# shamspias/fennec

Hardware: AMD Instinct MI355X
Metric: megapixels/sec: 4K SSIMFast+GaussianBlur (higher is better)
Workload: dtype u8 (blur: exact int32 sums of 24-bit fixed-point weights on the i8 matrix pipe; fp64 SSIM)

## Files before the change

fennec_amd/csrc/blur.hip:

```cpp
#include <hip/hip_ext.h>

#include "common.hpp"
#include "devutil.hpp"

#include <algorithm>
#include <cmath>

namespace fnx {

template <typename T>
struct PassArgs {
    const uint8_t *src;
    const uint8_t *const *srcs;
    const uint8_t *alpha;
    const uint8_t *const *alphas;
    uint8_t *dst;
    uint8_t *const *dsts;
    int sstride, astride, dstride, w, h, radius;
    const T *kern;
};

template <typename T> __device__ __forceinline__ T acc_tap(T acc, uint32_t v, T wt);
template <> __device__ __forceinline__ double acc_tap<double>(double acc, uint32_t v, double wt)
{
// ... 638 lines not shown

static bool guard_kernel_ok(const double *kernel, int radius)
{
    double sum = 0;
    for (int i = 0; i < 2 * radius + 1; i++) {
        if (!(kernel[i] >= 0)) return false;
        sum += kernel[i];
    }
    return sum <= 1.0 + 1e-9;
}

template <int R, bool SCORE, bool GUARD = false>
static int launch_direct(fnx_ctx *ctx, int n, FusedArgs &fa, bool tall)
{
    if constexpr (R > SCORE_RMAX) {
        static_assert(!SCORE, "one-pass form: R <= 8");
        return launch_direct_cfg<R, 256, WIDE_IH, false, GUARD>(ctx, n, fa);
    } else {
        constexpr int TH0 = ((64 - 2 * R) / 4) * 4;
        if (tall) return launch_direct_cfg<R, 256, 2 * TH0 + 2 * R, SCORE, GUARD>(ctx, n, fa);
        return launch_direct_cfg<R, 128, 64, SCORE, GUARD>(ctx, n, fa);
    }
}

template <bool SCORE, bool GUARD = false>
static int launch_direct_radius(fnx_ctx *ctx, int radius, int n, FusedArgs &fa, bool tall)
{
    switch (radius) {
    case 1: return launch_direct<1, SCORE, GUARD>(ctx, n, fa, tall);
    case 2: return launch_direct<2, SCORE, GUARD>(ctx, n, fa, tall);
    case 3: return launch_direct<3, SCORE, GUARD>(ctx, n, fa, tall);
    case 4: return launch_direct<4, SCORE, GUARD>(ctx, n, fa, tall);
    case 5: return launch_direct<5, SCORE, GUARD>(ctx, n, fa, tall);
    case 6: return launch_direct<6, SCORE, GUARD>(ctx, n, fa, tall);
    case 7: return launch_direct<7, SCORE, GUARD>(ctx, n, fa, tall);
    case 8: return launch_direct<8, SCORE, GUARD>(ctx, n, fa, tall);
    }
    if constexpr (!SCORE) {
        switch (radius) {
        case 9: return launch_direct<9, false, GUARD>(ctx, n, fa, tall);
        case 10: return launch_direct<10, false, GUARD>(ctx, n, fa, tall);
        case 11: return launch_direct<11, false, GUARD>(ctx, n, fa, tall);
        case 12: return launch_direct<12, false, GUARD>(ctx, n, fa, tall);
        case 13: return launch_direct<13, false, GUARD>(ctx, n, fa, tall);
        case 14: return launch_direct<14, false, GUARD>(ctx, n, fa, tall);
        case 15: return launch_direct<15, false, GUARD>(ctx, n, fa, tall);
        case 16: return launch_direct<16, false, GUARD>(ctx, n, fa, tall);
        }
    }
    return FNX_ERR_INVALID;
}

constexpr int NHEAD = 260 + 257 * 8;
static bool build_score_geom(fnx::ScoreGeom &g, int w, int h, int radius, int dstW, int dstH, int th_fixed = 0)
{
    if (radius < 1 || radius > (th_fixed ? 24 : SCORE_RMAX) || w < dstW || h < dstH || dstW <= 0 || dstH <= 0 || w >= (1 << 24) ||
        h >= (1 << 24))
        return false;
    const double xr = static_cast<double>(w) / static_cast<double>(dstW);
    const double yr = static_cast<double>(h) / static_cast<double>(dstH);
    if (std::fmin(xr, yr) < 3.6) return false;
    const size_t ref_words = 4 * (static_cast<size_t>(dstW) + dstH);
    std::vector<int32_t> &map = g.map;
    map.assign(NHEAD + ref_words + static_cast<size_t>(w) + h, -1);
    {
        uint32_t *magic = reinterpret_cast<uint32_t *>(map.data()), *tiedown = magic + 260;
        std::fill(magic, magic + NHEAD, 0u);
        for (uint32_t c = 1; c <= 256; c++) {
            magic[c] = static_cast<uint32_t>((1ull << 32) / (2ull * c)) + 1u;
            if (c & 1u) continue;
            const double inv = 1.0 / static_cast<double>(c);
            for (uint32_t k = 0; k < 256; k++) {
                const double n = static_cast<double>(c / 2) * static_cast<double>(2 * k + 1);
                if (n > 255.0 * c) break;
                if (n * inv < static_cast<double>(k) + 0.5) tiedown[8 * c + (k >> 5)] |= 1u << (k & 31);
            }
        }
    }
    BoxRef *xref = reinterpret_cast<BoxRef *>(map.data() + NHEAD), *yref = xref + dstW;
    int32_t *bx = map.data() + NHEAD + ref_words, *by = bx + w;
    int maxbw = 0, maxbh = 0;
    for (int d = 0; d < dstW; d++) {
        int s0, s1;
        box_edge(d, xr, w, s0, s1);
        if (d + 1 < dstW) { int n0, n1; box_edge(d + 1, xr, w, n0, n1); if (n0 < s1) return false; }
        for (int x = s0; x < s1; x++) bx[x] = d;
        if (s1 - s0 > maxbw) maxbw = s1 - s0;
    }
    for (int d = 0; d < dstH; d++) {
        int s0, s1;
        box_edge(d, yr, h, s0, s1);
        if (d + 1 < dstH) { int n0, n1; box_edge(d + 1, yr, h, n0, n1); if (n0 < s1) return false; }
        for (int y = s0; y < s1; y++) by[y] = d;
        if (s1 - s0 > maxbh) maxbh = s1 - s0;
    }
    if (static_cast<long>(maxbw) * maxbh > 256) return false;
    bool tall = g.tall_pref;
    int th = 0, nbx = 0, nby = 0;
    for (int attempt = 0; attempt < (th_fixed ? 1 : 2); attempt++, tall = !tall) {
        th = th_fixed ? th_fixed : direct_tile_rows(radius, tall);
        nbx = nby = 1;
        auto span = [](const int32_t *m, int lo, int hi) {
            int first = -1, last = -1;
            for (int i = lo; i < hi; i++)
                if (m[i] >= 0) { if (first < 0) first = m[i]; last = m[i]; }
            return first < 0 ? 0 : last - first + 1;
        };
        for (int x0 = 0; x0 < w; x0 += 64) nbx = std::max(nbx, span(bx, x0, std::min(w, x0 + 64)));
        for (int y0 = 0; y0 < h; y0 += th) nby = std::max(nby, span(by, y0, std::min(h, y0 + th)));
        if ((nbx + 1) * (nby + 1) <= (th_fixed > 272 ? 2 * SCORE_NBOX : SCORE_NBOX)) break;
        th = 0;
    }
    if (!th) return false;
    tall = th == direct_tile_rows(radius, true);
    if (th_fixed) {
        for (int x0 = 0; x0 < w; x0 += 16) {
            int first = -1, last = -1;
            for (int x = x0; x < std::min(w, x0 + 16); x++)
                if (bx[x] >= 0) { if (first < 0) first = bx[x]; last = bx[x]; }
            if (first >= 0 && last - first > 4) return false;
        }
    }
    for (int x0 = 0; x0 < w; x0 += 64)
        if (bx[x0] < 0) for (int x = x0; x < std::min(w, x0 + 64); x++) if (bx[x] >= 0) return false;
    for (int y0 = 0; y0 < h; y0 += th)
        if (by[y0] < 0) for (int y = y0; y < std::min(h, y0 + th); y++) if (by[y] >= 0) return false;

    const int slabn = (nbx + 1) * (nby + 1);
    const int tiles_x = (w + 63) / 64, tiles = tiles_x * ((h + th - 1) / th);
    if (static_cast<size_t>(tiles) * 2 * slabn >= (1u << 30)) return false;
    for (int d = 0; d < dstW; d++) {
        int s0, s1;
        box_edge(d, xr, w, s0, s1);
        const int t0 = s0 >> 6, t1 = (s1 - 1) >> 6;
        if (t1 > t0 + 1) return false;
        xref[d].part0 = t0 * 2 * slabn + (d - bx[t0 << 6]);
        xref[d].part1 = t1 > t0 ? t1 * 2 * slabn + (d - bx[t1 << 6]) : -1;
        xref[d].len = s1 - s0; xref[d].pad = 0;
    }
    for (int d = 0; d < dstH; d++) {
        int s0, s1;
        box_edge(d, yr, h, s0, s1);
        const int t0 = s0 / th, t1 = (s1 - 1) / th;
        if (t1 > t0 + 1) return false;
        yref[d].part0 = t0 * tiles_x * 2 * slabn + (d - by[t0 * th]) * (nbx + 1);
        yref[d].part1 = t1 > t0 ? t1 * tiles_x * 2 * slabn + (d - by[t1 * th]) * (nbx + 1) : -1;
        yref[d].len = s1 - s0; yref[d].pad = 0;
    }

    g.th = th; g.nbx = nbx; g.nby = nby; g.tall = tall;
    return true;
}

int launch_blur_scored(fnx_ctx *ctx, int n, const uint8_t *const *srcs, int sstride, int w, int h,
                       const double *kernel, int radius, int flags, uint8_t *const *dsts, int dstride,
                       uint8_t *planes, size_t plane, int dstW, int dstH)
{
    if (n > 65535) return FNX_NOOP;
    const bool exact = flags & FNX_BLUR_EXACT;
    const bool wide = radius > 6 && blur_mfma_wide_scored_covers(kernel, radius, w, h, exact);
    if (!wide) {
        if (radius < 1 || radius > SCORE_RMAX) return FNX_NOOP;
        if (exact && !guard_kernel_ok(kernel, radius)) return FNX_NOOP;
        if (radius > 6 && blur_mfma_takes(kernel, radius, w, h, exact)) return FNX_NOOP;
    }
    const bool tall_pref = wide ? false : direct_tall(ctx, radius, n, w, h);
    static const int wide_cap = [] { const char *e = dev_env("FNX_MFMA_WIDE_SEG"); return e ? atoi(e) : 544; }();
    const int seg = wide ? blur_mfma_segment(ctx, n, w, h, wide_cap, 2)
                         : (blur_mfma_covers(kernel, radius, w, h) && (!exact || blur_mfma_exact_enabled()) ? blur_mfma_segment(ctx, n, w, h, 272, 3) : 0);
    ScoreGeom &g = ctx->score_geom;
    if (!(g.w == w && g.h == h && g.dstW == dstW && g.dstH == dstH && g.radius == radius && g.tall_pref == tall_pref && g.seg == seg)) {
        g.w = w; g.h = h; g.dstW = dstW; g.dstH = dstH; g.radius = radius; g.tall_pref = tall_pref; g.seg = seg;
        g.mfma = seg > 0 && build_score_geom(g, w, h, radius, dstW, dstH, seg);
        g.ok = g.mfma || (!wide && seg == 0 && build_score_geom(g, w, h, radius, dstW, dstH));
    }
    if (!g.ok) return FNX_NOOP;
    const std::vector<int32_t> &map = g.map;
    const int th = g.th, nbx = g.nbx, nby = g.nby;
    const bool tall = g.tall;
    const size_t ref_words = 4 * (static_cast<size_t>(dstW) + dstH);
    const int slabn = (nbx + 1) * (nby + 1);
    const int tiles_x = (w + 63) / 64, tiles = tiles_x * ((h + th - 1) / th);

    void *dmap = nullptr;
    FNX_TRY(upload_table(ctx, SLOT_BOXMAP, map.data(), sizeof(int32_t) * map.size(), &dmap));
    FusedArgs fa{};
    fa.srcs = srcs; fa.dsts = dsts;
    fa.sstride = sstride; fa.dstride = dstride; fa.w = w; fa.h = h;
    for (int i = 0; i < 2 * radius + 1 && !wide; i++) {
        fa.wt[i] = static_cast<float>(kernel[i]);
        fa.wd[i] = kernel[i];
    }
    fa.bx = static_cast<const int32_t *>(dmap) + NHEAD + ref_words; fa.by = fa.bx + w;
    fa.nbx = nbx; fa.nby = nby;
    void *slabs = nullptr;
    FNX_TRY(scratch(ctx, ctx->parity ? SLOT_SLABS1 : SLOT_SLABS, sizeof(unsigned long long) * 2 * slabn * static_cast<size_t>(tiles) * n, &slabs));
    fa.slabs = static_cast<unsigned long long *>(slabs);
    int st;
    if (g.mfma) {
        st = wide ? launch_blur_mfma_wide_scored(ctx, n, srcs, sstride, w, h, kernel, radius, flags, dsts, dstride, fa.bx, fa.by, fa.slabs, nbx, nby, th)
                  : launch_blur_mfma_scored(ctx, n, srcs, sstride, w, h, kernel, radius, flags, dsts, dstride, fa.bx, fa.by, fa.slabs, nbx, nby, th);
        if (st == FNX_NOOP) return FNX_NOOP;
    } else {
        st = exact ? launch_direct_radius<true, true>(ctx, radius, n, fa, tall)
                   : launch_direct_radius<true, false>(ctx, radius, n, fa, tall);
    }
    if (st < 0) return st;
    hipStream_t box_stream = ctx->stream2;
    if (ctx->boxes_on_main) box_stream = ctx->stream;
    else {
        FNX_HIP(hipStreamWaitEvent(ctx->stream2, ctx->blur_done, 0));
        ctx->stream2_used = true;
    }

    SlabArgs sa{};
    sa.slabs = fa.slabs; sa.dst = planes; sa.plane = plane;
    sa.magic = static_cast<const uint32_t *>(dmap);
    sa.tiedown = sa.magic + 260;
    sa.xref = reinterpret_cast<const BoxRef *>(static_cast<const int32_t *>(dmap) + NHEAD);
    sa.yref = sa.xref + dstW;
    sa.image_slabs = static_cast<size_t>(tiles) * 2 * slabn;
    sa.n = n; sa.dstW = dstW; sa.dstH = dstH; sa.slabn = slabn;
    hipLaunchKernelGGL(box_from_slabs_kernel, dim3((dstW + 64 * BFS_BOXES - 1) / (64 * BFS_BOXES), (dstH + 3) / 4, n), dim3(256), 0,
                       box_stream, sa);
    FNX_HIP(hipGetLastError());
    return FNX_OK;
// ... 236 lines not shown
```

fennec_amd/csrc/blur_mfma.hip:

```cpp
#include <hip/hip_ext.h>

#include "common.hpp"
#include "devutil.hpp"

#include <algorithm>
#include <cmath>
#include <type_traits>
#include <vector>

namespace fnx {

typedef int v4i __attribute__((ext_vector_type(4)));

constexpr int MF_RMAX = 6;
constexpr int MF_P = 48;
constexpr int MF_WT = 64 * MF_P + 256;
constexpr int MF_SP = 352;
constexpr int MF_OP = 272;
constexpr int MF_SEG_SCORE = 272;
constexpr int MF_SEG_SCORE_WIDE = 544;

struct MfmaArgs {
    const uint8_t *src;
    const uint8_t *const *srcs;
    uint8_t *dst;
    uint8_t *const *dsts;
    int sstride, dstride, w, h;
    int tiles_x, tiles, seg;
    int radius;
    const uint32_t *tab;
    int seed_h, seed_v, thr;
    const int32_t *bx, *by;
    unsigned long long *slabs;
    int nbx, nby;
    int dbg;
};

__device__ __forceinline__ int mf_comb3(int hi, int mid, int lo)
{
    int t = hi * 256 + mid;
    asm volatile("" : "+v"(t));
    return t * 256 + lo;
}

__device__ __forceinline__ const double *mf_scalar_ptr(const double *p)
{
    const unsigned long long v = reinterpret_cast<unsigned long long>(p);
    const unsigned lo = __builtin_amdgcn_readfirstlane(static_cast<unsigned>(v)), hi = __builtin_amdgcn_readfirstlane(static_cast<unsigned>(v >> 32));
    return reinterpret_cast<const double *>((static_cast<unsigned long long>(hi) << 32) | lo);
}
typedef int mf_s16i __attribute__((ext_vector_type(16)));
__device__ __forceinline__ uint32_t mf_exact_u(const double *wd, const uint8_t *base, int step, int ring0, int mask)
{
    mf_s16i w0, w1;
    asm volatile("s_load_dwordx16 %0, %2, 0x0\n\ts_load_dwordx16 %1, %2, 0x40\n\ts_waitcnt lgkmcnt(0)" : "=&s"(w0), "=&s"(w1) : "s"(mf_scalar_ptr(wd)) : "memory");
    uint32_t v[13];
#pragma unroll
    for (int t = 0; t < 13; t++) v[t] = base[((ring0 + t) & mask) * step];
    double acc = 0;
#pragma unroll
    for (int t = 0; t < 13; t++) {
        const int lo = t < 8 ? w0[2 * (t & 7)] : w1[2 * (t & 7)], hi = t < 8 ? w0[2 * (t & 7) + 1] : w1[2 * (t & 7) + 1];
        acc = acc + u8_to_f64(v[t] ^ 0x80u) * __hiloint2double(hi, lo);
    }
    return clampF_dev(acc);
}

__device__ __forceinline__ void mf_box_add4(uint32_t *tbl, const u32x4 ro, uint32_t coln, const v4i cb)
{
#pragma unroll
    for (int k = 0; k < 4; k++)
        __hip_atomic_fetch_add(reinterpret_cast<uint32_t *>(reinterpret_cast<char *>(tbl) + ro[k] + coln), static_cast<uint32_t>(cb[k]),
                               __ATOMIC_RELAXED, __HIP_MEMORY_SCOPE_WORKGROUP);
}

template <bool SCORE, bool GUARD>
__global__ __launch_bounds__(256, GUARD ? 3 : 1) void blur_mfma_kernel(MfmaArgs a)
{
    constexpr int P = MF_P, WT = MF_WT, SP = MF_SP, OP = MF_OP;
    __shared__ __attribute__((aligned(16))) uint8_t s_t[4 * WT];
    __shared__ __attribute__((aligned(16))) uint8_t s_stage[2 * 16 * SP];
    __shared__ __attribute__((aligned(16))) uint8_t s_out[2 * 16 * OP];
    __shared__ __attribute__((aligned(16))) uint32_t s_rowh[SCORE ? MF_SEG_SCORE + 32 : 4];
    __shared__ __attribute__((aligned(16))) uint32_t s_rowv[SCORE ? MF_SEG_SCORE + 16 : 4];
    __shared__ uint32_t s_colbox[SCORE ? 64 : 1];
    extern __shared__ __attribute__((aligned(16))) uint32_t s_box[];

    const int tile = xcd_tile(blockIdx.x, a.tiles);
    if (tile < 0) return;
    const int z = blockIdx.y;
    const uint8_t *src = a.srcs ? a.srcs[z] : a.src;
    uint8_t *dst = a.dsts ? a.dsts[z] : a.dst;
    const int ty = tile / a.tiles_x, tx = tile - ty * a.tiles_x;
    const int x0 = tx * 64, y0 = ty * a.seg;
    const int tid = threadIdx.x, wave = tid >> 6, lane = tid & 63;
    const int r = lane & 15, g = lane >> 4;
    const int NJ = min(a.seg, ((a.h - y0 + 15) >> 4) << 4) >> 4;
    const int NI = NJ + 1;
    const bool xedge = x0 - 6 < 0 || x0 + 70 > a.w;

    const v4i *tbh = reinterpret_cast<const v4i *>(a.tab);
    const long *tbv = reinterpret_cast<const long *>(a.tab + 3 * 64 * 4);
    const v4i bh2 = tbh[lane], bh1 = tbh[64 + lane], bh0 = tbh[128 + lane];
    const long bv2 = tbv[lane], bv1 = tbv[64 + lane], bv0 = tbv[128 + lane];
    const bool alane = (r & 3) == 3;
    const int seed_hl = alane ? (1 << 23) + 128 : a.seed_h;
    const v4i sh = {seed_hl, seed_hl, seed_hl, seed_hl}, sv = {a.seed_v, a.seed_v, a.seed_v, a.seed_v};
    const v4i zero = {0, 0, 0, 0};
    const uint32_t sel01 = alane ? 0x0c0c0400u : 0x0c0c0703u, sel23 = alane ? 0x04000c0cu : 0x07030c0cu;

    uint8_t *tw = s_t + wave * WT;
    const int id1 = min(256 + tid, 16 * 19 - 1);
    const int srow0 = tid / 19, sch0 = tid - 19 * srow0, srow1 = id1 / 19, sch1 = id1 - 19 * srow1;
    const bool two = tid < 48;
    const int st_w0 = srow0 * SP + 16 * sch0, st_w1 = srow1 * SP + 16 * sch1;
    const int st_r = r * SP + 64 * wave + 16 * g;
    uint8_t *t_w = tw + r * P + 4 * g;
    const int m4 = r >> 2, mi = r & 3;
    const uint8_t *t_r = tw + (16 * m4 + mi) * P + 64 * m4 + 8 * g;
    const uint8_t *t_ro = tw + (16 * m4 + mi) * P + 64 * m4 + ((8 * g + 16) & 31);
    const uint8_t *t_ae = tw + (16 * g + 3) * P + 64 * g + r + 6;
    const uint8_t *t_ao = tw + (16 * g + 3) * P + 64 * g + ((r + 22) & 31);
    const int o_w = r * OP + 64 * wave + 16 * g;
    const int orow = tid >> 4, och = tid & 15;
    const int o_r = orow * OP + 16 * och;
    const int xo = x0 + 4 * och;

    v4i bbox = {0, 0, 0, 0}, sbox = {0, 0, 0, 0};
    uint32_t coln = 0;
    const int slabn = SCORE ? (a.nbx + 1) * (a.nby + 1) : 0;
    uint32_t *tbl_s = s_box, *tbl_b = s_box + 4 * slabn;
    auto score_setup = [&]() {
        if (!(a.dbg & 4)) for (int e = tid; e < 8 * slabn; e += 256) s_box[e] = 0;
        const int rowbytes = 16 * (a.nbx + 1);
        const int b0y = a.by[y0];
        for (int u = tid; u < 16 * NI; u += 256) {
            const int t = u - 6;
            const int v = (t >= 0 && t < a.seg && y0 + t < a.h) ? a.by[y0 + t] : -1;
            s_rowh[u] = rowbytes * ((v >= 0 && b0y >= 0) ? v - b0y : a.nby);
        }
        for (int t = tid; t < 16 * NJ; t += 256) {
            const int v = (t < a.seg && y0 + t < a.h) ? a.by[y0 + t] : -1;
            s_rowv[t] = rowbytes * ((v >= 0 && b0y >= 0) ? v - b0y : a.nby);
        }
        if (tid < 64) {
            const int b0x = a.bx[x0], v = x0 + tid < a.w ? a.bx[x0 + tid] : -1;
            s_colbox[tid] = (v >= 0 && b0x >= 0) ? v - b0x : 255u;
        }
        __syncthreads();
        uint32_t first = 255u;
        for (int i = 0; i < 16; i++) first = min(first, s_colbox[16 * wave + i]);
        const int slot = r / 3, ch = r - 3 * slot;
        int cnt = 0;
        for (int i = 0; i < 16; i++) cnt += (r < 15 && s_colbox[16 * wave + i] == first + slot) ? 1 : 0;
#pragma unroll
        for (int e = 0; e < 4; e++) {
            const bool in = r < 15 && first != 255u && s_colbox[16 * wave + 4 * g + e] == first + slot;
            bbox[e] = in ? (1 << (8 * ch)) : 0;
        }
        const int seed = 128 * cnt;
        sbox = (v4i){seed, seed, seed, seed};
        const uint32_t bc = (r < 15 && first != 255u && cnt > 0) ? first + slot : static_cast<uint32_t>(a.nbx);
        coln = 16u * bc + 4u * (r < 15 ? ch : 3);
    };

    const double *wd = reinterpret_cast<const double *>(a.tab + 3 * 64 * 4 + 3 * 64 * 2);

    auto stage_write = [&](const u32x4 (&d)[2], int buf) {
        uint8_t *sb = s_stage + buf * 16 * SP;
        *reinterpret_cast<u32x4 *>(sb + st_w0) = d[0] ^ 0x80808080u;
        if (two) *reinterpret_cast<u32x4 *>(sb + st_w1) = d[1] ^ 0x80808080u;
    };
    auto hset = [&](int s, int buf, int slot) {
        const uint8_t *sbuf = s_stage + buf * 16 * SP;
        const uint8_t *sb = sbuf + st_r;
        if constexpr (!GUARD && !SCORE) {
#pragma unroll
            for (int hf = 0; hf < 2; hf++) {
                v4i c2[2], c1[2], c0[2];
#pragma unroll
                for (int q2 = 0; q2 < 2; q2++) {
                    const v4i A = *reinterpret_cast<const v4i *>(sb + 16 * (2 * hf + q2));
                    c2[q2] = __builtin_amdgcn_mfma_i32_16x16x64_i8(A, bh2, zero, 0, 0, 0);
                    c1[q2] = __builtin_amdgcn_mfma_i32_16x16x64_i8(A, bh1, zero, 0, 0, 0);
                    c0[q2] = __builtin_amdgcn_mfma_i32_16x16x64_i8(A, bh0, sh, 0, 0, 0);
                }
#pragma unroll
                for (int q2 = 0; q2 < 2; q2++) {
                    const int qq = 2 * hf + q2;
                    v4i u;
#pragma unroll
                    for (int k = 0; k < 4; k++) u[k] = mf_comb3(c2[q2][k], c1[q2][k], c0[q2][k]);
                    const uint32_t t01 = __builtin_amdgcn_perm((uint32_t)u[1], (uint32_t)u[0], sel01);
                    const uint32_t t23 = __builtin_amdgcn_perm((uint32_t)u[3], (uint32_t)u[2], sel23);
                    *reinterpret_cast<uint32_t *>(t_w + (16 * qq) * P + 64 * qq + 16 * slot) = t01 | t23;
                }
                __builtin_amdgcn_sched_barrier(0);
            }
            return;
        }
        v4i c2[4], c1[4], c0[4];
#pragma unroll
        for (int qq = 0; qq < 4; qq++) {
            const v4i A = *reinterpret_cast<const v4i *>(sb + 16 * qq);
            c2[qq] = __builtin_amdgcn_mfma_i32_16x16x64_i8(A, bh2, zero, 0, 0, 0);
            c1[qq] = __builtin_amdgcn_mfma_i32_16x16x64_i8(A, bh1, zero, 0, 0, 0);
            c0[qq] = __builtin_amdgcn_mfma_i32_16x16x64_i8(A, bh0, sh, 0, 0, 0);
        }
        if constexpr (SCORE) {
            const u32x2 lo = *reinterpret_cast<const u32x2 *>(sb + 24), hi = *reinterpret_cast<const u32x2 *>(sb + 32);
            const v4i A = {(int)lo.x, (int)lo.y, (int)hi.x, (int)hi.y};
            const v4i cb = __builtin_amdgcn_mfma_i32_16x16x64_i8(A, bbox, sbox, 0, 0, 0);
            const u32x4 ro = *reinterpret_cast<const u32x4 *>(s_rowh + 16 * s + 4 * g);
            if (!(a.dbg & 1)) mf_box_add4(tbl_s, ro, coln, cb);
        }
        v4i u[4];
#pragma unroll
        for (int qq = 0; qq < 4; qq++)
#pragma unroll
            for (int k = 0; k < 4; k++) u[qq][k] = mf_comb3(c2[qq][k], c1[qq][k], c0[qq][k]);
#pragma unroll
        for (int qq = 0; qq < 4; qq++) {
            const uint32_t t01 = __builtin_amdgcn_perm((uint32_t)u[qq][1], (uint32_t)u[qq][0], sel01);
            const uint32_t t23 = __builtin_amdgcn_perm((uint32_t)u[qq][3], (uint32_t)u[qq][2], sel23);
            *reinterpret_cast<uint32_t *>(t_w + (16 * qq) * P + 64 * qq + 16 * slot) = t01 | t23;
        }
        if constexpr (GUARD) {
            uint32_t m[4];
#pragma unroll
            for (int qq = 0; qq < 4; qq++) {
                const uint32_t f0 = static_cast<uint32_t>(u[qq][0]) & 0x00ffffffu, f1 = static_cast<uint32_t>(u[qq][1]) & 0x00ffffffu;
                const uint32_t f2 = static_cast<uint32_t>(u[qq][2]) & 0x00ffffffu, f3 = static_cast<uint32_t>(u[qq][3]) & 0x00ffffffu;
                m[qq] = min(min(min(f0, f1), f2), f3);
            }
            const uint32_t mm = min(min(min(m[0], m[1]), m[2]), m[3]);
            if (__builtin_amdgcn_ballot_w64(mm < static_cast<uint32_t>(a.thr))) {
                uint32_t fl = 0;
#pragma unroll
                for (int qq = 0; qq < 4; qq++)
#pragma unroll
                    for (int k = 0; k < 4; k++) fl |= ((static_cast<uint32_t>(u[qq][k]) & 0x00ffffffu) < static_cast<uint32_t>(a.thr) ? 1u : 0u) << (4 * qq + k);
                unsigned long long todo = __builtin_amdgcn_ballot_w64(fl != 0);
                while (todo) {
                    const int L = __builtin_ctzll(todo);
                    todo &= todo - 1;
                    uint32_t flL = __builtin_amdgcn_readlane(fl, L);
                    const int rL = L & 15, gL = L >> 4;
                    while (flL) {
                        const int b = __builtin_ctz(flL), qq = b >> 2, k = b & 3;
                        flL &= flL - 1;
                        const uint32_t e = mf_exact_u(wd, sbuf + (4 * gL + k) * SP + 4 * (16 * wave + 4 * qq + (rL >> 2)) + (rL & 3), 4, 0, 0xffff) ^ 0x80u;
                        if (lane == L) *(t_w + (16 * qq) * P + 64 * qq + 16 * slot + k) = static_cast<uint8_t>(e);
                    }
                }
            }
        }
    };
    auto vset = [&](int j, int buf, auto oddt) {
        constexpr bool ODD = decltype(oddt)::value;
        long A[4];
        uint32_t al[4];
#pragma unroll
        for (int q = 0; q < 4; q++) A[q] = *reinterpret_cast<const long *>((ODD ? t_ro : t_r) + (4 * q) * P);
#pragma unroll
        for (int q = 0; q < 4; q++) al[q] = *((ODD ? t_ao : t_ae) + (4 * q) * P);
        int u[4][3];
        if constexpr (!GUARD && !SCORE) {
// ... 17 lines not shown
#pragma unroll
            for (int q = 0; q < 4; q++) {
                c2[q] = __builtin_amdgcn_mfma_i32_16x16x32_i8(A[q], bv2, zero, 0, 0, 0);
                c1[q] = __builtin_amdgcn_mfma_i32_16x16x32_i8(A[q], bv1, zero, 0, 0, 0);
                c0[q] = __builtin_amdgcn_mfma_i32_16x16x32_i8(A[q], bv0, sv, 0, 0, 0);
            }
#pragma unroll
            for (int q = 0; q < 4; q++)
#pragma unroll
                for (int i = 0; i < 3; i++) u[q][i] = mf_comb3(c2[q][i], c1[q][i], c0[q][i]);
        }
        u32x4 o;
#pragma unroll
        for (int q = 0; q < 4; q++) {
            const uint32_t t01 = __builtin_amdgcn_perm((uint32_t)u[q][1], (uint32_t)u[q][0], 0x0c0c0703u);
            const uint32_t t23 = __builtin_amdgcn_perm(al[q], (uint32_t)u[q][2], 0x04030c0cu);
            o[q] = t01 | t23;
        }
        uint8_t *op = s_out + buf * 16 * OP + o_w;
        *reinterpret_cast<u32x4 *>(op) = o;
        if constexpr (GUARD) {
            uint32_t m[4];
#pragma unroll
            for (int q = 0; q < 4; q++)
                m[q] = min(min(static_cast<uint32_t>(u[q][0]) & 0x00ffffffu, static_cast<uint32_t>(u[q][1]) & 0x00ffffffu), static_cast<uint32_t>(u[q][2]) & 0x00ffffffu);
            const uint32_t mm = min(min(min(m[0], m[1]), m[2]), m[3]);
            if (__builtin_amdgcn_ballot_w64(mm < static_cast<uint32_t>(a.thr))) {
                uint32_t fl = 0;
#pragma unroll
                for (int q = 0; q < 4; q++)
#pragma unroll
                    for (int i = 0; i < 3; i++) fl |= ((static_cast<uint32_t>(u[q][i]) & 0x00ffffffu) < static_cast<uint32_t>(a.thr) ? 1u : 0u) << (4 * q + i);
                unsigned long long todo = __builtin_amdgcn_ballot_w64(fl != 0);
                while (todo) {
                    const int L = __builtin_ctzll(todo);
                    todo &= todo - 1;
                    uint32_t flL = __builtin_amdgcn_readlane(fl, L);
                    const int rL = L & 15, gL = L >> 4;
                    while (flL) {
                        const int b = __builtin_ctz(flL), q = b >> 2, i = b & 3;
                        flL &= flL - 1;
                        const uint32_t e = mf_exact_u(wd, tw + (16 * gL + 4 * q + i) * P + 64 * gL, 1, (ODD ? 16 : 0) + rL, 31);
                        if (lane == L) op[4 * q + i] = static_cast<uint8_t>(e);
                    }
                }
                if constexpr (SCORE) o = *reinterpret_cast<const u32x4 *>(op);
            }
        }
        if constexpr (SCORE) {
            const u32x4 os = o ^ 0x80808080u;
            const v4i A = {(int)os[0], (int)os[1], (int)os[2], (int)os[3]};
            const v4i cb = __builtin_amdgcn_mfma_i32_16x16x64_i8(A, bbox, sbox, 0, 0, 0);
            const u32x4 ro = *reinterpret_cast<const u32x4 *>(s_rowv + 16 * j + 4 * g);
            if (!(a.dbg & 1)) mf_box_add4(tbl_b, ro, coln, cb);
        }
    };

    auto march = [&](auto xedget) {
        constexpr bool XEDGE = decltype(xedget)::value;
        auto hload = [&](int i, u32x4 (&d)[2]) {
            const int ys = y0 - 6 + 16 * i;
            if constexpr (!XEDGE) {
                const uint8_t *sb = src + 4 * static_cast<ptrdiff_t>(x0 - 6);
                const int ya = clampi(ys + srow0, 0, a.h - 1), yb = clampi(ys + srow1, 0, a.h - 1);
                d[0] = *(g_u32x4 *)(sb + static_cast<ptrdiff_t>(ya) * a.sstride + 16 * sch0);
                d[1] = *(g_u32x4 *)(sb + static_cast<ptrdiff_t>(yb) * a.sstride + 16 * sch1);
            } else {
    #pragma unroll
                for (int k = 0; k < 2; k++) {
                    if (k == 1 && !two) break;
                    const int y = clampi(ys + (k ? srow1 : srow0), 0, a.h - 1);
                    const uint8_t *rowp = src + static_cast<size_t>(y) * a.sstride;
                    const int xc = x0 - 6 + 4 * (k ? sch1 : sch0);
    #pragma unroll
                    for (int e = 0; e < 4; e++) d[k][e] = ld_px(rowp, clampi(xc + e, 0, a.w - 1));
                }
            }
        };
        auto out_store = [&](int j, int buf) {
            const u32x4 o = *reinterpret_cast<const u32x4 *>(s_out + buf * 16 * OP + o_r);
            const int y = y0 + 16 * j + orow;
            if (y < a.h) {
                uint8_t *dp = dst + static_cast<size_t>(y) * a.dstride + 4 * static_cast<size_t>(xo);
                if (!XEDGE || xo + 3 < a.w) *(g_u32x4w *)(dp) = o;
                else {
    #pragma unroll
                    for (int e = 0; e < 4; e++) if (xo + e < a.w) *(g_u32w *)(dp + 4 * e) = o[e];
                }
            }
        };
        u32x4 ra[2], rb[2];
        hload(0, ra);
        __builtin_amdgcn_sched_barrier(0);
        hload(min(1, NI - 1), rb);
        __builtin_amdgcn_sched_barrier(0);
        if constexpr (SCORE) score_setup();
        auto step = [&](int s, u32x4 (&d)[2], auto oddv) {
            constexpr int par = decltype(oddv)::value ? 0 : 1;
            if (s < NI) stage_write(d, par);
            if (XEDGE) { if (s + 2 < NI) hload(s + 2, d); } else hload(min(s + 2, NI - 1), d);
            if (s >= 3 && s - 3 < NJ) out_store(s - 3, par);
            __syncthreads();
            if (s < NI) hset(s, par, par);
            if (s >= 1 && s - 1 < NJ) vset(s - 1, par, oddv);
        };
    #pragma unroll 1
        for (int s = 0; s < NJ + 3; s += 2) {
            step(s, ra, std::true_type{});
            step(s + 1, rb, std::false_type{});
        }

    };
    if (xedge) march(std::true_type{}); else march(std::false_type{});

    if (SCORE && !(a.dbg & 2)) {
        __syncthreads();
        unsigned long long *slab = a.slabs + (static_cast<size_t>(z) * a.tiles + tile) * 2 * slabn;
        for (int e = tid; e < 2 * slabn; e += 256) {
            const u32x4 v = *reinterpret_cast<const u32x4 *>(s_box + 4 * e);
            slab[e] = static_cast<unsigned long long>(v.x | (v.y << 16)) | (static_cast<unsigned long long>(v.z) << 32);
        }
    }
}

template <int NKH> struct MfWide {
    static constexpr int NKV = NKH <= 4 ? 1 : (NKH <= 7 ? 2 : 3);
    static constexpr int RFH = 8 * NKH - 2, RFV = 32 * NKV - 8;
    static constexpr int RF = RFH < RFV ? RFH : RFV;
    static constexpr int NC = 16 + RF / 2;
    static constexpr int NL = (16 * NC + 255) / 256;
    static constexpr int SP = 16 * NC + 48;
    static constexpr int NT = 2 * RF + 1;
    static constexpr int NS = 4 * NKV;
    static constexpr int RING = 16 * NS;
    static constexpr int P = RING + 16;
    static constexpr int WT = 64 * P + 256;
};

template <int NT>
__device__ __noinline__ uint32_t mf_exact_h_n(const uint8_t *p, const double *wd)
{
    double acc = 0;
#pragma unroll 15
    for (int t = 0; t < NT; t++) acc = acc + u8_to_f64(p[4 * t] ^ 0x80u) * wd[t];
    return clampF_dev(acc);
}
template <int NT, int RING = 64>
__device__ __noinline__ uint32_t mf_exact_v_n(const uint8_t *p, int ring0, const double *wd)
{
    double acc = 0;
#pragma unroll 15
    for (int t = 0; t < NT; t++) acc = acc + u8_to_f64(p[static_cast<unsigned>(ring0 + t) % static_cast<unsigned>(RING)] ^ 0x80u) * wd[t];
    return clampF_dev(acc);
}

template <int NT>
__device__ __forceinline__ uint32_t mf_exact_u_n(const double *wd, const uint8_t *base, int step, int ring0, int mask)
{
    double acc = 0;
#pragma unroll
    for (int t0 = 0; t0 < NT; t0 += 8) {
        mf_s16i w;
        asm volatile("s_load_dwordx16 %0, %1, %2\n\ts_waitcnt lgkmcnt(0)" : "=&s"(w) : "s"(mf_scalar_ptr(wd)), "n"(8 * t0) : "memory");
        uint32_t v[8];
#pragma unroll
        for (int t = 0; t < 8; t++) v[t] = base[((ring0 + t0 + min(t, NT - 1 - t0)) & mask) * step];
#pragma unroll
        for (int t = 0; t < 8; t++)
            if (t0 + t < NT) acc = acc + u8_to_f64(v[t] ^ 0x80u) * __hiloint2double(w[2 * t + 1], w[2 * t]);
    }
    return clampF_dev(acc);
}

// ... 531 lines not shown
    FNX_TRY(prof_bind(ctx, FNX_PROF_MAIN, &ev));
    if constexpr (SCORE) {
        if (!ev.stop) ev.stop = ctx->ev_blur[ctx->parity];
        ctx->blur_done = ev.stop;
        note_route(ctx, FNX_PROF_MAIN, exact ? "blur_mfma_wide_kernel<SCORE, GUARD>" : "blur_mfma_wide_kernel<SCORE>");
    } else {
        note_route(ctx, FNX_PROF_MAIN, exact ? "blur_mfma_wide_kernel<GUARD>" : "blur_mfma_wide_kernel");
    }
    if (exact) hipExtLaunchKernelGGL((blur_mfma_wide_kernel<NKH, true, SCORE>), grid, dim3(256), lds, ctx->stream, ev.start, ev.stop, 0, ma);
    else hipExtLaunchKernelGGL((blur_mfma_wide_kernel<NKH, false, SCORE>), grid, dim3(256), lds, ctx->stream, ev.start, ev.stop, 0, ma);
    FNX_HIP(hipGetLastError());
    return FNX_OK;
}

int launch_blur_mfma(fnx_ctx *ctx, int n, const uint8_t *src, const uint8_t *const *srcs, int sstride, int w, int h,
                     const double *kernel, int radius, int flags, uint8_t *dst, uint8_t *const *dsts, int dstride)
{
    const bool exact = flags & FNX_BLUR_EXACT;
    if (exact && !blur_mfma_exact_enabled()) return FNX_NOOP;
    if (n > 65535) return FNX_NOOP;
    if (blur_mfma_wide_covers(kernel, radius, w, h)) {
        MfmaWeights q;
        mfma_quantise(kernel, radius, &q, MF_RWIDE);
        const long long gq = exact ? static_cast<long long>(std::ceil(q.err255)) + 2 : 0;
        if (gq > (1 << 20)) return FNX_NOOP;
        MfmaArgs ma{};
        ma.src = src; ma.srcs = srcs; ma.dst = dst; ma.dsts = dsts;
        ma.sstride = sstride; ma.dstride = dstride; ma.w = w; ma.h = h;
        ma.seed_h = static_cast<int>((1u << 23) + static_cast<uint32_t>(gq));
        ma.seed_v = static_cast<int>((1u << 23) + (1u << 31) + static_cast<uint32_t>(gq));
        ma.thr = static_cast<int>(2 * gq);
        ma.seg = blur_mfma_segment(ctx, n, w, h, 544, 3);
        if (radius <= MfWide<2>::RF) return launch_mfma_wide<2>(ctx, n, ma, q, kernel, radius, exact);
        if (radius <= MfWide<3>::RF) return launch_mfma_wide<3>(ctx, n, ma, q, kernel, radius, exact);
        if (radius > MfWide<4>::RF) {
            if (radius <= MfWide<5>::RF) return launch_mfma_wide<5>(ctx, n, ma, q, kernel, radius, exact);
            if (radius <= MfWide<6>::RF) return launch_mfma_wide<6>(ctx, n, ma, q, kernel, radius, exact);
            if (radius <= MfWide<7>::RF) return launch_mfma_wide<7>(ctx, n, ma, q, kernel, radius, exact);
            return launch_mfma_wide<8>(ctx, n, ma, q, kernel, radius, exact);
        }
        return launch_mfma_wide<4>(ctx, n, ma, q, kernel, radius, exact);
    }
    if (!blur_mfma_covers(kernel, radius, w, h)) return FNX_NOOP;
    MfmaArgs ma{};
    const int st = mfma_prepare(ctx, kernel, radius, exact, &ma);
    if (st != FNX_OK) return st;
    ma.src = src; ma.srcs = srcs; ma.dst = dst; ma.dsts = dsts;
    ma.sstride = sstride; ma.dstride = dstride; ma.w = w; ma.h = h;
    static const int cap = [] { const char *e = dev_env("FNX_MFMA_SEG"); return e ? atoi(e) : 544; }();
    ma.seg = blur_mfma_segment(ctx, n, w, h, cap, exact ? 3 : 4);
    return exact ? launch_mfma_cfg<false, true>(ctx, n, ma, 0) : launch_mfma_cfg<false, false>(ctx, n, ma, 0);
}

int launch_blur_mfma_scored(fnx_ctx *ctx, int n, const uint8_t *const *srcs, int sstride, int w, int h, const double *kernel,
                            int radius, int flags, uint8_t *const *dsts, int dstride, const int32_t *bx, const int32_t *by,
                            unsigned long long *slabs, int nbx, int nby, int seg)
{
    const bool exact = flags & FNX_BLUR_EXACT;
    MfmaArgs ma{};
    const int st = mfma_prepare(ctx, kernel, radius, exact, &ma);
    if (st != FNX_OK) return st;
    ma.srcs = srcs; ma.dsts = dsts;
    ma.sstride = sstride; ma.dstride = dstride; ma.w = w; ma.h = h;
    ma.seg = seg;
    ma.bx = bx; ma.by = by; ma.slabs = slabs; ma.nbx = nbx; ma.nby = nby;
    const size_t lds = sizeof(uint32_t) * 8 * static_cast<size_t>(nbx + 1) * (nby + 1);
    return exact ? launch_mfma_cfg<true, true>(ctx, n, ma, lds) : launch_mfma_cfg<true, false>(ctx, n, ma, lds);
}

bool blur_mfma_wide_scored_covers(const double *kernel, int radius, int w, int h, bool exact)
{
    if (radius > MfWide<4>::RF || (exact && !blur_mfma_exact_enabled())) return false;
    return blur_mfma_wide_covers(kernel, radius, w, h);
}
int launch_blur_mfma_wide_scored(fnx_ctx *ctx, int n, const uint8_t *const *srcs, int sstride, int w, int h, const double *kernel,
                                 int radius, int flags, uint8_t *const *dsts, int dstride, const int32_t *bx, const int32_t *by,
                                 unsigned long long *slabs, int nbx, int nby, int seg)
{
    const bool exact = flags & FNX_BLUR_EXACT;
    if (!blur_mfma_wide_scored_covers(kernel, radius, w, h, exact) || seg > MF_SEG_SCORE_WIDE) return FNX_NOOP;
    MfmaWeights q;
    mfma_quantise(kernel, radius, &q, MF_RWIDE);
    const long long gq = exact ? static_cast<long long>(std::ceil(q.err255)) + 2 : 0;
    if (gq > (1 << 20)) return FNX_NOOP;
    MfmaArgs ma{};
    ma.srcs = srcs; ma.dsts = dsts;
    ma.sstride = sstride; ma.dstride = dstride; ma.w = w; ma.h = h;
    ma.seed_h = static_cast<int>((1u << 23) + static_cast<uint32_t>(gq));
    ma.seed_v = static_cast<int>((1u << 23) + (1u << 31) + static_cast<uint32_t>(gq));
    ma.thr = static_cast<int>(2 * gq);
    ma.seg = seg;
    ma.bx = bx; ma.by = by; ma.slabs = slabs; ma.nbx = nbx; ma.nby = nby;
    const size_t lds = sizeof(uint32_t) * 8 * static_cast<size_t>(nbx + 1) * (nby + 1);
    if (radius <= MfWide<2>::RF) return launch_mfma_wide<2, true>(ctx, n, ma, q, kernel, radius, exact, lds);
    if (radius <= MfWide<3>::RF) return launch_mfma_wide<3, true>(ctx, n, ma, q, kernel, radius, exact, lds);
    return launch_mfma_wide<4, true>(ctx, n, ma, q, kernel, radius, exact, lds);
}

}

extern "C" int fnx_blur_fixed_point(const double *kernel, int radius, long long *wq, double *err255)
{
    if (!kernel || !wq || !err255) {
        fnx::set_error("invalid argument: fnx_blur_fixed_point");
        return FNX_ERR_INVALID;
    }
    fnx::MfmaWeights q;
    if (!fnx::mfma_quantise(kernel, radius, &q, fnx::MF_RWIDE)) return FNX_NOOP;
    for (int i = 0; i < 2 * radius + 1; i++) wq[i] = q.wq[i];
    *err255 = q.err255;
    return FNX_OK;
}
```

fennec_amd/csrc/common.hpp:

```cpp
#pragma once
#include <hip/hip_runtime.h>

#include <cstdarg>
#include <cstdint>
#include <cstdio>
#include <cstdlib>
#include <cstring>
#include <vector>

#include "../../include/fennec_hip.h"

namespace fnx {

void set_error(const char *fmt, ...);

#ifdef FNX_DEVELOP
inline const char *dev_env(const char *name) { return std::getenv(name); }
#else
inline const char *dev_env(const char *) { return nullptr; }
#endif

enum Form {
    FORM_FX_STREAM = 0,
    FORM_FX_PAIRS,
// ... 207 lines not shown
    uint8_t *host = nullptr;
    int hstride = 0, w = 0, h = 0;
};

int stage_in(fnx_ctx *ctx, int space, const uint8_t *src, int sstride, int w, int h, Slot slot,
             DevImg *out);
int stage_in_flat(fnx_ctx *ctx, int space, const uint8_t *src, int sstride, int w, int h, Slot slot,
                  DevImg *out);
int stage_in_front(fnx_ctx *ctx, int space, const uint8_t *src, int w, int h, Slot slot, DevImg *out);
int stage_out(fnx_ctx *ctx, int space, uint8_t *dst, int dstride, int w, int h, Slot slot,
              DevOut *out);
int finish(fnx_ctx *ctx, int space, DevOut *out);
int finish_enqueue(fnx_ctx *ctx, int space, DevOut *out);
struct LaunchEvents {
    hipEvent_t start = nullptr, stop = nullptr;
};
int prof_bind(fnx_ctx *ctx, int cls, LaunchEvents *ev);
int prof_begin(fnx_ctx *ctx, int cls = FNX_PROF_MAIN);
inline void note_route(fnx_ctx *ctx, int cls, const char *kernel)
{
    int i = 0;
    while (i < 7 && !((cls >> i) & 1)) i++;
    ctx->route[i] = kernel;
}
int prof_end(fnx_ctx *ctx);
int fetch_doubles(fnx_ctx *ctx, const double *dptr, double *host, int n);
int fetch_bytes(fnx_ctx *ctx, const void *dptr, void *host, size_t bytes);

inline bool aligned16(const void *p, int stride)
{
    return ((reinterpret_cast<uintptr_t>(p) | static_cast<uintptr_t>(stride)) & 15u) == 0;
}

int check_img(const void *p, int stride, int w, int h, const char *what);
int check_space(int space);
int check_space_io(int space);
bool ssim_fast_dims(int w, int h, int *nw, int *nh);
int result_slot(fnx_ctx *ctx, int n, double **d);
int result_wait(fnx_ctx *ctx, const double *pinned, double *out, int n);
int against_device(fnx_ctx *ctx, const fnx_prepared *ref, const uint8_t *b, int bstride, const double *window, double *out,
                   bool b_is_plane = false);
int prepared_plane(fnx_ctx *ctx, const uint8_t *src, int sstride, const fnx_prepared &ref);

int launch_blur(fnx_ctx *ctx, int n, const uint8_t *src, const uint8_t *const *srcs, int sstride,
                int w, int h, const double *kernel, int radius, int flags, uint8_t *dst,
                uint8_t *const *dsts, int dstride);
int launch_blur_scored(fnx_ctx *ctx, int n, const uint8_t *const *srcs, int sstride, int w, int h,
                       const double *kernel, int radius, int flags, uint8_t *const *dsts, int dstride,
                       uint8_t *planes, size_t plane, int dstW, int dstH);
bool blur_mfma_covers(const double *kernel, int radius, int w, int h);
bool blur_mfma_exact_enabled();
bool blur_mfma_takes(const double *kernel, int radius, int w, int h, bool exact);
int blur_mfma_segment(const fnx_ctx *ctx, int n, int w, int h, int cap, int occ);
int launch_blur_mfma(fnx_ctx *ctx, int n, const uint8_t *src, const uint8_t *const *srcs, int sstride, int w, int h,
                     const double *kernel, int radius, int flags, uint8_t *dst, uint8_t *const *dsts, int dstride);
int launch_blur_mfma_scored(fnx_ctx *ctx, int n, const uint8_t *const *srcs, int sstride, int w, int h, const double *kernel,
                            int radius, int flags, uint8_t *const *dsts, int dstride, const int32_t *bx, const int32_t *by,
                            unsigned long long *slabs, int nbx, int nby, int seg);
bool blur_mfma_wide_scored_covers(const double *kernel, int radius, int w, int h, bool exact);
int launch_blur_mfma_wide_scored(fnx_ctx *ctx, int n, const uint8_t *const *srcs, int sstride, int w, int h, const double *kernel,
                                 int radius, int flags, uint8_t *const *dsts, int dstride, const int32_t *bx, const int32_t *by,
                                 unsigned long long *slabs, int nbx, int nby, int seg);
int launch_blur3x3(fnx_ctx *ctx, const uint8_t *src, int sstride, int w, int h, uint8_t *dst,
                   int dstride);
int launch_sharpen(fnx_ctx *ctx, bool adaptive, const uint8_t *src, int sstride, int w, int h,
                   double amount, uint8_t *dst, int dstride);
int launch_sharpen_batch(fnx_ctx *ctx, bool adaptive, int n, const uint8_t *src0, const uint8_t *const *d_srcs, int sstride, int w, int h,
                         double amount, uint8_t *dst0, uint8_t *const *d_dsts, int dstride);
struct ResizeHint {
    uint32_t *cells = nullptr;
    size_t cap = 0;
    int gx = 0, gy = 0, rows = 0;
    bool valid = false;
};
int resize_pass(fnx_ctx *ctx, bool vertical, const TapTable &t, const uint8_t *src, int sstride, int srcW, int srcH,
                uint8_t *dst, int dstride, ResizeHint *hint = nullptr);
int resize_fused(fnx_ctx *ctx, const TapTable &th, const TapTable &tv, const uint8_t *src, int sstride, int srcW, int srcH,
                 uint8_t *dst, int dstride, int nimg = 1, const uint8_t *const *d_srcs = nullptr, uint8_t *const *d_dsts = nullptr);
void free_resize_plans(fnx_ctx *ctx);
struct RzMfTable {
    bool ok = false;
    int KH = 0;
    int NC = 0;
    int ngroups = 0;
    int nmat = 0;
    int S = 22;
    int seed = 0, thr = 0;
    void *blob = nullptr;
    const void *mats = nullptr;
    const int32_t *meta = nullptr, *sbase = nullptr;
    const void *ex = nullptr;
};
bool resize_mfma_build(const fnx_ctx *ctx, const TapTable &t, int srcN, bool vertical, const double *inv, RzMfTable *out);
void resize_mfma_free(RzMfTable *t);
int resize_mfma_launch(fnx_ctx *ctx, const RzMfTable &h, const RzMfTable &v,
                       const uint8_t *src, int sstride, int srcW, int srcH, uint8_t *dst, int dstride, int dstW, int dstH,
                       uint32_t *todo, unsigned *gave_up, uint32_t gen, int old_tw, int old_th, int old_gx, int *workgroups,
                       int nimg = 1, const uint8_t *const *d_srcs = nullptr, uint8_t *const *d_dsts = nullptr, uint32_t todo_stride = 0);
int lanczos_resize_tables(fnx_ctx *ctx, int space, const uint8_t *src, int sstride, int srcW, int srcH,
                          const TapTable &th, const TapTable &tv, uint8_t *dst, int dstride, int dstW, int dstH);
int lanczos_resize_tables_batch(fnx_ctx *ctx, int n, const uint8_t *const *srcs, int sstride, int srcW, int srcH,
                                const TapTable &th, const TapTable &tv, uint8_t *const *dsts, int dstride, int dstW, int dstH);
int launch_resize_h(fnx_ctx *ctx, const uint8_t *src, int sstride, int srcW, int srcH,
                    const int32_t *d_off, const int32_t *d_idx, const double *d_wt, uint8_t *dst,
                    int dstride, int dstW, int contig_taps);
int resize_contiguous_taps(const int32_t *off, const int32_t *idx, int nout);
// ... 124 lines not shown
```

Measured before the change: 402,500.

## Pack scored-blur box table into shared rows and allow taller MFMA segments

Repacks the per-tile LDS box-sum table so source and blurred sums share one 32-bit word per channel, with the blurred value shifted into the upper 16 bits. The row layout becomes 3 words per box plus padding. The smaller table lets the non-wide scored MFMA path take segments up to 544 rows instead of 272, and a fallback loop retries smaller segment caps when the geometry does not fit. The aim is fewer tiles, less halo recomputation and less LDS per block. The risk is 16-bit overflow in packed sums and lower occupancy from taller tiles.

```diff
diff --git a/fennec_amd/csrc/blur.hip b/fennec_amd/csrc/blur.hip
--- a/fennec_amd/csrc/blur.hip
+++ b/fennec_amd/csrc/blur.hip
@@ -714,7 +714,8 @@
 }
 
 constexpr int NHEAD = 260 + 257 * 8;
-static bool build_score_geom(fnx::ScoreGeom &g, int w, int h, int radius, int dstW, int dstH, int th_fixed = 0)
+static bool build_score_geom(fnx::ScoreGeom &g, int w, int h, int radius, int dstW, int dstH, int th_fixed = 0,
+                             bool (*fits)(int nbx, int nby) = nullptr)
 {
     if (radius < 1 || radius > (th_fixed ? 24 : SCORE_RMAX) || w < dstW || h < dstH || dstW <= 0 || dstH <= 0 || w >= (1 << 24) ||
         h >= (1 << 24))
@@ -770,7 +771,7 @@
         };
         for (int x0 = 0; x0 < w; x0 += 64) nbx = std::max(nbx, span(bx, x0, std::min(w, x0 + 64)));
         for (int y0 = 0; y0 < h; y0 += th) nby = std::max(nby, span(by, y0, std::min(h, y0 + th)));
-        if ((nbx + 1) * (nby + 1) <= (th_fixed > 272 ? 2 * SCORE_NBOX : SCORE_NBOX)) break;
+        if (fits ? fits(nbx, nby) : (nbx + 1) * (nby + 1) <= SCORE_NBOX) break;
         th = 0;
     }
     if (!th) return false;
@@ -827,13 +828,20 @@
         if (radius > 6 && blur_mfma_takes(kernel, radius, w, h, exact)) return FNX_NOOP;
     }
     const bool tall_pref = wide ? false : direct_tall(ctx, radius, n, w, h);
+    const int score_cap = blur_mfma_score_seg_cap();
     static const int wide_cap = [] { const char *e = dev_env("FNX_MFMA_WIDE_SEG"); return e ? atoi(e) : 544; }();
     const int seg = wide ? blur_mfma_segment(ctx, n, w, h, wide_cap, 2)
-                         : (blur_mfma_covers(kernel, radius, w, h) && (!exact || blur_mfma_exact_enabled()) ? blur_mfma_segment(ctx, n, w, h, 272, 3) : 0);
+                         : (blur_mfma_covers(kernel, radius, w, h) && (!exact || blur_mfma_exact_enabled()) ? blur_mfma_segment(ctx, n, w, h, score_cap, 3) : 0);
     ScoreGeom &g = ctx->score_geom;
     if (!(g.w == w && g.h == h && g.dstW == dstW && g.dstH == dstH && g.radius == radius && g.tall_pref == tall_pref && g.seg == seg)) {
         g.w = w; g.h = h; g.dstW = dstW; g.dstH = dstH; g.radius = radius; g.tall_pref = tall_pref; g.seg = seg;
-        g.mfma = seg > 0 && build_score_geom(g, w, h, radius, dstW, dstH, seg);
+        bool (*const wide_fits)(int, int) = seg > 272 ? +[](int bx, int by) { return (bx + 1) * (by + 1) <= 2 * SCORE_NBOX; } : nullptr;
+        g.mfma = seg > 0 && build_score_geom(g, w, h, radius, dstW, dstH, seg, wide ? wide_fits : blur_mfma_score_fits);
+        for (int cap = score_cap - 16, last = seg; cap >= 16 && !g.mfma && seg > 0 && !wide; cap -= 16) {
+            const int s = blur_mfma_segment(ctx, n, w, h, cap, 3);
+            if (s != last) g.mfma = build_score_geom(g, w, h, radius, dstW, dstH, s, blur_mfma_score_fits);
+            last = s;
+        }
         g.ok = g.mfma || (!wide && seg == 0 && build_score_geom(g, w, h, radius, dstW, dstH));
     }
     if (!g.ok) return FNX_NOOP;
diff --git a/fennec_amd/csrc/blur_mfma.hip b/fennec_amd/csrc/blur_mfma.hip
--- a/fennec_amd/csrc/blur_mfma.hip
+++ b/fennec_amd/csrc/blur_mfma.hip
@@ -17,7 +17,9 @@
 constexpr int MF_WT = 64 * MF_P + 256;
 constexpr int MF_SP = 352;
 constexpr int MF_OP = 272;
-constexpr int MF_SEG_SCORE = 272;
+constexpr int MF_SEG_SCORE = 544;
+constexpr int MF_SCORE_TABLE_BYTES = 15360;
+__host__ __device__ constexpr int mf_score_row_words(int nbx) { return 3 * nbx + 16; }
 constexpr int MF_SEG_SCORE_WIDE = 544;
 
 struct MfmaArgs {
@@ -66,11 +68,12 @@
     return clampF_dev(acc);
 }
 
+template <int SHIFT = 0>
 __device__ __forceinline__ void mf_box_add4(uint32_t *tbl, const u32x4 ro, uint32_t coln, const v4i cb)
 {
 #pragma unroll
     for (int k = 0; k < 4; k++)
-        __hip_atomic_fetch_add(reinterpret_cast<uint32_t *>(reinterpret_cast<char *>(tbl) + ro[k] + coln), static_cast<uint32_t>(cb[k]),
+        __hip_atomic_fetch_add(reinterpret_cast<uint32_t *>(reinterpret_cast<char *>(tbl) + ro[k] + coln), static_cast<uint32_t>(cb[k]) << SHIFT,
                                __ATOMIC_RELAXED, __HIP_MEMORY_SCOPE_WORKGROUP);
 }
 
@@ -129,10 +132,9 @@
     v4i bbox = {0, 0, 0, 0}, sbox = {0, 0, 0, 0};
     uint32_t coln = 0;
     const int slabn = SCORE ? (a.nbx + 1) * (a.nby + 1) : 0;
-    uint32_t *tbl_s = s_box, *tbl_b = s_box + 4 * slabn;
     auto score_setup = [&]() {
-        if (!(a.dbg & 4)) for (int e = tid; e < 8 * slabn; e += 256) s_box[e] = 0;
-        const int rowbytes = 16 * (a.nbx + 1);
+        if (!(a.dbg & 4)) for (int e = tid; e < (a.nby + 1) * mf_score_row_words(a.nbx); e += 256) s_box[e] = 0;
+        const int rowbytes = 4 * mf_score_row_words(a.nbx);
         const int b0y = a.by[y0];
         for (int u = tid; u < 16 * NI; u += 256) {
             const int t = u - 6;
@@ -160,8 +162,8 @@
         }
         const int seed = 128 * cnt;
         sbox = (v4i){seed, seed, seed, seed};
-        const uint32_t bc = (r < 15 && first != 255u && cnt > 0) ? first + slot : static_cast<uint32_t>(a.nbx);
-        coln = 16u * bc + 4u * (r < 15 ? ch : 3);
+        const bool boxed = r < 15 && first != 255u && cnt > 0;
+        coln = boxed ? 12u * (first + slot) + 4u * ch : 12u * a.nbx + 4u * r;
     };
 
     const double *wd = reinterpret_cast<const double *>(a.tab + 3 * 64 * 4 + 3 * 64 * 2);
@@ -212,7 +214,7 @@
             const v4i A = {(int)lo.x, (int)lo.y, (int)hi.x, (int)hi.y};
             const v4i cb = __builtin_amdgcn_mfma_i32_16x16x64_i8(A, bbox, sbox, 0, 0, 0);
             const u32x4 ro = *reinterpret_cast<const u32x4 *>(s_rowh + 16 * s + 4 * g);
-            if (!(a.dbg & 1)) mf_box_add4(tbl_s, ro, coln, cb);
+            if (!(a.dbg & 1)) mf_box_add4<0>(s_box, ro, coln, cb);
         }
         v4i u[4];
 #pragma unroll
@@ -336,7 +338,7 @@
             const v4i A = {(int)os[0], (int)os[1], (int)os[2], (int)os[3]};
             const v4i cb = __builtin_amdgcn_mfma_i32_16x16x64_i8(A, bbox, sbox, 0, 0, 0);
             const u32x4 ro = *reinterpret_cast<const u32x4 *>(s_rowv + 16 * j + 4 * g);
-            if (!(a.dbg & 1)) mf_box_add4(tbl_b, ro, coln, cb);
+            if (!(a.dbg & 1)) mf_box_add4<16>(s_box, ro, coln, cb);
         }
     };
 
@@ -400,9 +402,12 @@
     if (SCORE && !(a.dbg & 2)) {
         __syncthreads();
         unsigned long long *slab = a.slabs + (static_cast<size_t>(z) * a.tiles + tile) * 2 * slabn;
-        for (int e = tid; e < 2 * slabn; e += 256) {
-            const u32x4 v = *reinterpret_cast<const u32x4 *>(s_box + 4 * e);
-            slab[e] = static_cast<unsigned long long>(v.x | (v.y << 16)) | (static_cast<unsigned long long>(v.z) << 32);
+        for (int row = tid >> 5, col = tid & 31; row <= a.nby && col <= a.nbx; row += 8) {
+            const int e = row * (a.nbx + 1) + col;
+            const uint32_t *pe = s_box + row * mf_score_row_words(a.nbx) + 3 * col;
+            const uint32_t vr = pe[0], vg = pe[1], vb = pe[2];
+            slab[e] = static_cast<unsigned long long>((vr & 0xffffu) | (vg << 16)) | (static_cast<unsigned long long>(vb & 0xffffu) << 32);
+            slab[slabn + e] = static_cast<unsigned long long>((vr >> 16) | (vg & 0xffff0000u)) | (static_cast<unsigned long long>(vb >> 16) << 32);
         }
     }
 }
@@ -1040,6 +1045,12 @@
     return exact ? launch_mfma_cfg<false, true>(ctx, n, ma, 0) : launch_mfma_cfg<false, false>(ctx, n, ma, 0);
 }
 
+int blur_mfma_score_seg_cap() { return MF_SEG_SCORE; }
+bool blur_mfma_score_fits(int nbx, int nby)
+{
+    return nbx + 1 <= 32 && static_cast<long>(nby + 1) * 4 * mf_score_row_words(nbx) <= MF_SCORE_TABLE_BYTES;
+}
+
 int launch_blur_mfma_scored(fnx_ctx *ctx, int n, const uint8_t *const *srcs, int sstride, int w, int h, const double *kernel,
                             int radius, int flags, uint8_t *const *dsts, int dstride, const int32_t *bx, const int32_t *by,
                             unsigned long long *slabs, int nbx, int nby, int seg)
@@ -1052,7 +1063,8 @@
     ma.sstride = sstride; ma.dstride = dstride; ma.w = w; ma.h = h;
     ma.seg = seg;
     ma.bx = bx; ma.by = by; ma.slabs = slabs; ma.nbx = nbx; ma.nby = nby;
-    const size_t lds = sizeof(uint32_t) * 8 * static_cast<size_t>(nbx + 1) * (nby + 1);
+    if (seg > MF_SEG_SCORE || !blur_mfma_score_fits(nbx, nby)) return FNX_NOOP;
+    const size_t lds = sizeof(uint32_t) * mf_score_row_words(nbx) * static_cast<size_t>(nby + 1);
     return exact ? launch_mfma_cfg<true, true>(ctx, n, ma, lds) : launch_mfma_cfg<true, false>(ctx, n, ma, lds);
 }
 
diff --git a/fennec_amd/csrc/common.hpp b/fennec_amd/csrc/common.hpp
--- a/fennec_amd/csrc/common.hpp
+++ b/fennec_amd/csrc/common.hpp
@@ -283,6 +283,8 @@
 bool blur_mfma_exact_enabled();
 bool blur_mfma_takes(const double *kernel, int radius, int w, int h, bool exact);
 int blur_mfma_segment(const fnx_ctx *ctx, int n, int w, int h, int cap, int occ);
+int blur_mfma_score_seg_cap();
+bool blur_mfma_score_fits(int nbx, int nby);
 int launch_blur_mfma(fnx_ctx *ctx, int n, const uint8_t *src, const uint8_t *const *srcs, int sstride, int w, int h,
                      const double *kernel, int radius, int flags, uint8_t *dst, uint8_t *const *dsts, int dstride);
 int launch_blur_mfma_scored(fnx_ctx *ctx, int n, const uint8_t *const *srcs, int sstride, int w, int h, const double *kernel,
```

New measurement: 418,800 (median of 6 runs). 1.04x the previous value.
